# kmaninis/OSVOS-PyTorch

Measured on NVIDIA H100. Metric: frames/sec at 480x854 fwd-only, batch 1 per GPU (OSVOS.forward -> 5 logit maps), higher is better.
Workload: dtype bf16x3 (split-bf16 operands, fp32 accumulate)

## Files before the change

osvos_pytorch_b200/csrc/conv_stage1_fused.cu:

```cuda
#include <stdlib.h>
#include <string.h>

#include "conv_common.cuh"

namespace osvos {

constexpr int kS1Pitch = 10;
constexpr int kS1HaloRows = kTileH + 2;
constexpr int kS1HaloPx = kS1HaloRows * kS1Pitch;
constexpr int kS1APlane = (kS1HaloPx * 128 + 1023) / 1024 * 1024;
constexpr int kS1AStage = 2 * kS1APlane;
constexpr int kS1AStages = 2;
constexpr int kS1BPlane = 64 * 128;
constexpr int kS1BStage = 2 * kS1BPlane;
constexpr int kS1BStages = 5;
constexpr int kS1W1Bytes = (64 * 27 + 64) * 4;
constexpr int kS1Builders = 96;
constexpr int kS1Smem = kS1AStages * kS1AStage + kS1BStages * kS1BStage + kS1W1Bytes + 1024 + 512;
static_assert(kS1Smem <= 227 * 1024, "stage-1 kernel exceeds the per-CTA shared memory");
static_assert(kS1Smem + 4096 < (1 << 18), "descriptor start-address field would overflow");

struct Stage1Params {
  const float* x;
  const float* w1;
  const float* b1;
};

__global__ void __launch_bounds__(kConvThreads, 1)
conv_stage1_fused_kernel(const __grid_constant__ CUtensorMap map_w_hi, const __grid_constant__ CUtensorMap map_w_lo,
                         const Stage1Params s1, const ConvParams p) {
  extern __shared__ uint8_t smem_raw[];
  uint8_t* smem = reinterpret_cast<uint8_t*>((reinterpret_cast<uintptr_t>(smem_raw) + 1023) & ~uintptr_t(1023));
  uint8_t* smem_a = smem;
  uint8_t* smem_b = smem_a + kS1AStages * kS1AStage;
  float* w1s = reinterpret_cast<float*>(smem_b + kS1BStages * kS1BStage);
  uint64_t* bars = reinterpret_cast<uint64_t*>(reinterpret_cast<uint8_t*>(w1s) + kS1W1Bytes);
  uint64_t* a_full = bars;
  uint64_t* a_empty = bars + 2;
  uint64_t* b_full = bars + 4;
  uint64_t* b_empty = bars + 4 + kS1BStages;

  const int warp = threadIdx.x >> 5;
  const int lane = threadIdx.x & 31;

  if (threadIdx.x == 0) {
    tma_prefetch_desc(&map_w_hi);
    tma_prefetch_desc(&map_w_lo);
    for (int i = 0; i < 2; ++i) {
      mbar_init(&a_full[i], kS1Builders);
      mbar_init(&a_empty[i], 2);
    }
    for (int i = 0; i < kS1BStages; ++i) {
      mbar_init(&b_full[i], 1);
      mbar_init(&b_empty[i], 2);
    }
    fence_barrier_init();
  }
  pdl_wait();
  pdl_launch_dependents();
  for (int i = threadIdx.x; i < 64 * 27 + 64; i += kConvThreads)
    w1s[i] = i < 64 * 27 ? __ldg(s1.w1 + i) : (s1.b1 ? __ldg(s1.b1 + i - 64 * 27) : 0.f);
  __syncthreads();

  if (warp == 0) {
    if (elect_one()) {
      int b_stage = 0;
      uint32_t b_phase = 0;
      for (int tile = blockIdx.x; tile < p.total_tiles; tile += gridDim.x) {
#pragma unroll
        for (int tap = 0; tap < 9; ++tap) {
          mbar_wait(&b_empty[b_stage], b_phase ^ 1);
          uint8_t* st = smem_b + b_stage * kS1BStage;
          mbar_arrive_expect_tx(&b_full[b_stage], kS1BStage);
          tma_load_3d(&map_w_hi, &b_full[b_stage], st, 0, 0, tap);
          tma_load_3d(&map_w_lo, &b_full[b_stage], st + kS1BPlane, 0, 0, tap);
          if (++b_stage == kS1BStages) {
            b_stage = 0;
            b_phase ^= 1;
          }
        }
      }
    }
    __syncwarp();
  } else if (warp < 4) {
    const int t = threadIdx.x - 32;
    const size_t plane_sz = static_cast<size_t>(p.h) * p.w;
    int a_stage = 0;
    uint32_t a_phase = 0;
    for (int tile = blockIdx.x; tile < p.total_tiles; tile += gridDim.x) {
      int nb, tx, ty, img;
      decode_tile(p, tile, nb, tx, ty, img);
      mbar_wait(&a_empty[a_stage], a_phase ^ 1);
      uint8_t* st = smem_a + a_stage * kS1AStage;
      for (int pix = t; pix < kS1HaloPx; pix += kS1Builders) {
        const int hy = pix / kS1Pitch, hx = pix - hy * kS1Pitch;
        const int y = ty * kTileH - 1 + hy, xx = tx * kTileW - 1 + hx;
        const bool inside = y >= 0 && y < p.h && xx >= 0 && xx < p.w;
        float v[27];
#pragma unroll
        for (int ci = 0; ci < 3; ++ci) {
          const float* pl = s1.x + (static_cast<size_t>(img) * 3 + ci) * plane_sz;
#pragma unroll
          for (int r = 0; r < 3; ++r) {
            const int iy = y + r - 1;
#pragma unroll
            for (int s = 0; s < 3; ++s) {
              const int ix = xx + s - 1;
              v[ci * 9 + r * 3 + s] =
                  (inside && iy >= 0 && iy < p.h && ix >= 0 && ix < p.w) ? __ldg(pl + static_cast<size_t>(iy) * p.w + ix) : 0.f;
            }
          }
        }
#pragma unroll 1
        for (int chunk = 0; chunk < 8; ++chunk) {
          float f[8];
#pragma unroll
          for (int e = 0; e < 8; ++e) {
            const int co = chunk * 8 + e;
            float acc = w1s[64 * 27 + co];
#pragma unroll
            for (int k = 0; k < 27; ++k) acc = fmaf(w1s[co * 27 + k], v[k], acc);
            f[e] = inside ? fmaxf(acc, 0.f) : 0.f;
          }
          uint32_t hi[4], lo[4];
#pragma unroll
          for (int e = 0; e < 4; ++e) split_pack2(f[2 * e], f[2 * e + 1], hi[e], lo[e]);
          const uint32_t off = sw128_offset(pix, chunk);
          *reinterpret_cast<uint4*>(st + off) = make_uint4(hi[0], hi[1], hi[2], hi[3]);
          *reinterpret_cast<uint4*>(st + kS1APlane + off) = make_uint4(lo[0], lo[1], lo[2], lo[3]);
        }
      }
      fence_proxy_async_smem();
      mbar_arrive(&a_full[a_stage]);
      if (++a_stage == kS1AStages) {
        a_stage = 0;
        a_phase ^= 1;
      }
    }
  } else {
    const int wg = (warp - 4) >> 2, wl = warp & 3;
    const bool leader = (threadIdx.x & 127) == 0;
    constexpr uint64_t kDescA = desc_template(16, kS1Pitch * 128, kDescSW128);
    constexpr uint64_t kDescB = desc_template(16, 1024, kDescSW128);
    const uint32_t smem_a_u32 = smem_u32(smem_a) + wg * 8 * kS1Pitch * 128, smem_b_u32 = smem_u32(smem_b);
    float acc[64];
    int a_stage = 0, b_stage = 0;
    uint32_t a_phase = 0, b_phase = 0;
    StageRelease pending;
    for (int tile = blockIdx.x; tile < p.total_tiles; tile += gridDim.x) {
#pragma unroll
      for (int i = 0; i < 64; ++i) acc[i] = 0.f;
      mbar_wait(&a_full[a_stage], a_phase);
      const uint64_t da0 = kDescA | static_cast<uint64_t>((smem_a_u32 + a_stage * kS1AStage) >> 4);
#pragma unroll
      for (int tap = 0; tap < 9; ++tap) {
        const uint32_t tap_off = static_cast<uint32_t>(((tap / 3) * kS1Pitch + (tap % 3)) * (128 >> 4));
        mbar_wait(&b_full[b_stage], b_phase);
        const uint64_t db_hi = kDescB | static_cast<uint64_t>((smem_b_u32 + b_stage * kS1BStage) >> 4);
        const uint64_t da_hi = da0 + tap_off;
        const uint64_t da_lo = da_hi + (kS1APlane >> 4);
        wgmma_fence();
#pragma unroll
        for (int k = 0; k < kBlockK / 16; ++k) {
          wgmma_bf16<128>(acc, da_hi + 2 * k, db_hi + 2 * k, 1);
          wgmma_bf16<64>(acc, da_lo + 2 * k, db_hi + 2 * k, 1);
        }
        wgmma_commit();
        wgmma_wait<1>();
        pending.release(leader);
        pending.bar_b = &b_empty[b_stage];
        if (tap == 8) pending.bar_a = &a_empty[a_stage];
        if (++b_stage == kS1BStages) {
          b_stage = 0;
          b_phase ^= 1;
        }
      }
      if (++a_stage == kS1AStages) {
        a_stage = 0;
        a_phase ^= 1;
      }
      wgmma_wait<0>();
      wgmma_fence_operands(acc);
      pending.release(leader);
      conv_epilogue<64, true, true>(p, acc, tile, wg, wl, lane);
    }
  }
}

}

using namespace osvos;

extern "C" int osvos_stage1_fused(const osvos_stage1_args* a, osvos_stream_t stream_) {
  OSVOS_CHECK_ARG(a != nullptr && a->x != nullptr && a->w1 != nullptr && a->w2_packed != nullptr);
  OSVOS_CHECK_ARG(a->n > 0 && a->h > 0 && a->w > 0 && a->h <= 65535 && a->n <= 65535);
  OSVOS_CHECK_ARG((a->y_hi != nullptr && a->y_lo != nullptr) || (a->pool_hi != nullptr && a->pool_lo != nullptr));
  OSVOS_CHECK_ARG((a->y_hi == nullptr) == (a->y_lo == nullptr) && (a->pool_hi == nullptr) == (a->pool_lo == nullptr));
  {
    const uintptr_t any = reinterpret_cast<uintptr_t>(a->y_hi) | reinterpret_cast<uintptr_t>(a->y_lo) |
                          reinterpret_cast<uintptr_t>(a->pool_hi) | reinterpret_cast<uintptr_t>(a->pool_lo);
    OSVOS_CHECK_ARG((any & 3) == 0);
    OSVOS_CHECK_ARG(((reinterpret_cast<uintptr_t>(a->b1) | reinterpret_cast<uintptr_t>(a->b2) |
                      reinterpret_cast<uintptr_t>(a->w2_packed)) & 15) == 0);
  }
  cudaStream_t stream = static_cast<cudaStream_t>(stream_);
  osvos_conv3x3_args c;
  memset(&c, 0, sizeof(c));
  c.w_packed = a->w2_packed;
  c.bias = a->b2;
  c.y_hi = a->y_hi;
  c.y_lo = a->y_lo;
  c.pool_hi = a->pool_hi;
  c.pool_lo = a->pool_lo;
  c.n = a->n, c.h = a->h, c.w = a->w, c.cin = 64, c.cout = 64;
  c.flags = OSVOS_FLAG_RELU;
  ConvParams p;
  fill_conv_params(p, &c, 64);
  CUtensorMap mw_hi, mw_lo;
  int rc = encode_weight_maps(&mw_hi, &mw_lo, &c, 64);
  if (rc) return rc;
  Stage1Params s1;
  s1.x = a->x;
  s1.w1 = a->w1;
  s1.b1 = a->b1;
  const int sms = device_sm_count();
  const int grid = p.total_tiles < sms ? p.total_tiles : sms;
  auto kern = conv_stage1_fused_kernel;
  static uint64_t attr_done = 0;
  OSVOS_CHECK_CUDA(ensure_dynamic_smem(kern, kS1Smem, &attr_done));
  OSVOS_CHECK_CUDA(launch_pdl(kern, dim3(grid), dim3(kConvThreads), kS1Smem, stream, mw_hi, mw_lo, s1, p));
  return OSVOS_OK;
}
```

Before: 656.0.

## Compute conv1_1 on tensor cores inside consumer warpgroups with ping-pong tiles

Replaces the scalar-FMA builder warps that computed the 3-channel first convolution with a register-sourced wgmma (split bf16x3) inside each consumer warpgroup. The two consumer warpgroups now alternate whole tiles, ping-pong style, and are sequenced through named barriers. Producer warps give up registers via setmaxnreg, and the B pipeline grows to 7 stages. The aim is to remove the CUDA-core FMA bottleneck of building the halo activations, at the cost of more complex synchronisation and ablation flags in the hot path.

```diff
diff --git a/osvos_pytorch_b200/csrc/conv_stage1_fused.cu b/osvos_pytorch_b200/csrc/conv_stage1_fused.cu
--- a/osvos_pytorch_b200/csrc/conv_stage1_fused.cu
+++ b/osvos_pytorch_b200/csrc/conv_stage1_fused.cu
@@ -8,17 +8,19 @@
 constexpr int kS1Pitch = 10;
 constexpr int kS1HaloRows = kTileH + 2;
 constexpr int kS1HaloPx = kS1HaloRows * kS1Pitch;
+constexpr int kS1Blocks = (kS1HaloPx + 63) / 64;
 constexpr int kS1APlane = (kS1HaloPx * 128 + 1023) / 1024 * 1024;
 constexpr int kS1AStage = 2 * kS1APlane;
 constexpr int kS1AStages = 2;
 constexpr int kS1BPlane = 64 * 128;
 constexpr int kS1BStage = 2 * kS1BPlane;
-constexpr int kS1BStages = 5;
-constexpr int kS1W1Bytes = (64 * 27 + 64) * 4;
-constexpr int kS1Builders = 96;
+constexpr int kS1BStages = 7;
+constexpr int kS1W1Bytes = 2 * 64 * 128;
 constexpr int kS1Smem = kS1AStages * kS1AStage + kS1BStages * kS1BStage + kS1W1Bytes + 1024 + 512;
 static_assert(kS1Smem <= 227 * 1024, "stage-1 kernel exceeds the per-CTA shared memory");
 static_assert(kS1Smem + 4096 < (1 << 18), "descriptor start-address field would overflow");
+static_assert(kS1AStage % 1024 == 0 && kS1BStage % 1024 == 0 && kS1W1Bytes % 1024 == 0,
+              "operands keep 1024-byte alignment");
 
 struct Stage1Params {
   const float* x;
@@ -26,19 +28,37 @@
   const float* b1;
 };
 
+__device__ __forceinline__ void wgmma_bf16_rs64(float* d, const uint32_t (&a)[4], uint64_t desc_b, uint32_t scale_d) {
+  asm volatile(
+      "{\n.reg .pred p;\nsetp.ne.b32 p, %37, 0;\n"
+      "wgmma.mma_async.sync.aligned.m64n64k16.f32.bf16.bf16 {%0, %1, %2, %3, %4, %5, %6, %7, %8, %9, %10, %11, %12, %13, "
+      "%14, %15, %16, %17, %18, %19, %20, %21, %22, %23, %24, %25, %26, %27, %28, %29, %30, %31}, {%32, %33, %34, %35}, "
+      "%36, p, 1, 1, 0;\n}\n"
+      : "+f"(d[0]), "+f"(d[1]), "+f"(d[2]), "+f"(d[3]), "+f"(d[4]), "+f"(d[5]), "+f"(d[6]), "+f"(d[7]), "+f"(d[8]),
+        "+f"(d[9]), "+f"(d[10]), "+f"(d[11]), "+f"(d[12]), "+f"(d[13]), "+f"(d[14]), "+f"(d[15]), "+f"(d[16]),
+        "+f"(d[17]), "+f"(d[18]), "+f"(d[19]), "+f"(d[20]), "+f"(d[21]), "+f"(d[22]), "+f"(d[23]), "+f"(d[24]),
+        "+f"(d[25]), "+f"(d[26]), "+f"(d[27]), "+f"(d[28]), "+f"(d[29]), "+f"(d[30]), "+f"(d[31])
+      : "r"(a[0]), "r"(a[1]), "r"(a[2]), "r"(a[3]), "l"(desc_b), "r"(scale_d)
+      : "memory");
+}
+
+__device__ __forceinline__ void pin_regs(uint32_t (&r)[4]) {
+#pragma unroll
+  for (int i = 0; i < 4; ++i) asm volatile("" : "+r"(r[i])::"memory");
+}
+
 __global__ void __launch_bounds__(kConvThreads, 1)
 conv_stage1_fused_kernel(const __grid_constant__ CUtensorMap map_w_hi, const __grid_constant__ CUtensorMap map_w_lo,
                          const Stage1Params s1, const ConvParams p) {
+  constexpr int SB = kS1BStages;
   extern __shared__ uint8_t smem_raw[];
   uint8_t* smem = reinterpret_cast<uint8_t*>((reinterpret_cast<uintptr_t>(smem_raw) + 1023) & ~uintptr_t(1023));
   uint8_t* smem_a = smem;
   uint8_t* smem_b = smem_a + kS1AStages * kS1AStage;
-  float* w1s = reinterpret_cast<float*>(smem_b + kS1BStages * kS1BStage);
-  uint64_t* bars = reinterpret_cast<uint64_t*>(reinterpret_cast<uint8_t*>(w1s) + kS1W1Bytes);
-  uint64_t* a_full = bars;
-  uint64_t* a_empty = bars + 2;
-  uint64_t* b_full = bars + 4;
-  uint64_t* b_empty = bars + 4 + kS1BStages;
+  uint8_t* smem_w1 = smem_b + SB * kS1BStage;
+  uint64_t* bars = reinterpret_cast<uint64_t*>(smem_w1 + kS1W1Bytes);
+  uint64_t* b_full = bars;
+  uint64_t* b_empty = bars + SB;
 
   const int warp = threadIdx.x >> 5;
   const int lane = threadIdx.x & 31;
@@ -46,35 +66,54 @@
   if (threadIdx.x == 0) {
     tma_prefetch_desc(&map_w_hi);
     tma_prefetch_desc(&map_w_lo);
-    for (int i = 0; i < 2; ++i) {
-      mbar_init(&a_full[i], kS1Builders);
-      mbar_init(&a_empty[i], 2);
-    }
-    for (int i = 0; i < kS1BStages; ++i) {
+    for (int i = 0; i < SB; ++i) {
       mbar_init(&b_full[i], 1);
-      mbar_init(&b_empty[i], 2);
+      mbar_init(&b_empty[i], 1);
     }
     fence_barrier_init();
   }
   pdl_wait();
   pdl_launch_dependents();
-  for (int i = threadIdx.x; i < 64 * 27 + 64; i += kConvThreads)
-    w1s[i] = i < 64 * 27 ? __ldg(s1.w1 + i) : (s1.b1 ? __ldg(s1.b1 + i - 64 * 27) : 0.f);
+  for (int i = threadIdx.x; i < 64 * 4; i += kConvThreads) {
+    const int co = i >> 2, chunk = i & 3;
+    uint32_t hi[4], lo[4];
+#pragma unroll
+    for (int t = 0; t < 4; ++t) {
+      const int k0 = chunk * 8 + 2 * t;
+      const float v0 = k0 < 27 ? s1.w1[co * 27 + k0] : 0.f;
+      const float v1 = k0 + 1 < 27 ? s1.w1[co * 27 + k0 + 1] : 0.f;
+      __nv_bfloat16 h0, l0, h1, l1;
+      split_bf16(v0, h0, l0);
+      split_bf16(v1, h1, l1);
+      hi[t] = pack_bf16x2(h0, h1);
+      lo[t] = pack_bf16x2(l0, l1);
+    }
+    *reinterpret_cast<uint4*>(smem_w1 + sw128_offset(co, chunk)) = make_uint4(hi[0], hi[1], hi[2], hi[3]);
+    *reinterpret_cast<uint4*>(smem_w1 + 64 * 128 + sw128_offset(co, chunk)) = make_uint4(lo[0], lo[1], lo[2], lo[3]);
+  }
+  fence_proxy_async_smem();
   __syncthreads();
 
-  if (warp == 0) {
+  if (warp < 4) {
+    setmaxnreg_dec<40>();
+    if (warp != 0) return;
     if (elect_one()) {
+      const bool skip_b = (p.ablate & 1) != 0;
       int b_stage = 0;
       uint32_t b_phase = 0;
       for (int tile = blockIdx.x; tile < p.total_tiles; tile += gridDim.x) {
 #pragma unroll
         for (int tap = 0; tap < 9; ++tap) {
           mbar_wait(&b_empty[b_stage], b_phase ^ 1);
-          uint8_t* st = smem_b + b_stage * kS1BStage;
-          mbar_arrive_expect_tx(&b_full[b_stage], kS1BStage);
-          tma_load_3d(&map_w_hi, &b_full[b_stage], st, 0, 0, tap);
-          tma_load_3d(&map_w_lo, &b_full[b_stage], st + kS1BPlane, 0, 0, tap);
-          if (++b_stage == kS1BStages) {
+          if (skip_b) {
+            mbar_arrive(&b_full[b_stage]);
+          } else {
+            uint8_t* st = smem_b + b_stage * kS1BStage;
+            mbar_arrive_expect_tx(&b_full[b_stage], kS1BStage);
+            tma_load_3d(&map_w_hi, &b_full[b_stage], st, 0, 0, tap);
+            tma_load_3d(&map_w_lo, &b_full[b_stage], st + kS1BPlane, 0, 0, tap);
+          }
+          if (++b_stage == SB) {
             b_stage = 0;
             b_phase ^= 1;
           }
@@ -82,108 +121,166 @@
       }
     }
     __syncwarp();
-  } else if (warp < 4) {
-    const int t = threadIdx.x - 32;
-    const size_t plane_sz = static_cast<size_t>(p.h) * p.w;
-    int a_stage = 0;
-    uint32_t a_phase = 0;
-    for (int tile = blockIdx.x; tile < p.total_tiles; tile += gridDim.x) {
+    return;
+  }
+  setmaxnreg_inc<232>();
+  const int wg = (warp - 4) >> 2, wl = warp & 3;
+  const int t = threadIdx.x & 127;
+  const bool leader = t == 0;
+  const int build_bar = 3 + wg;
+  const bool skip_build = (p.ablate & 2) != 0, skip_mma = (p.ablate & 4) != 0;
+  uint8_t* stage = smem_a + wg * kS1AStage;
+  const uint32_t stage_u32 = smem_u32(stage);
+  const uint64_t dw1_hi = make_smem_desc(smem_w1, 16, 1024, kDescSW128), dw1_lo = dw1_hi + ((64 * 128) >> 4);
+  constexpr uint64_t kDescA = desc_template(16, kS1Pitch * 128, kDescSW128);
+  constexpr uint64_t kDescB = desc_template(16, 1024, kDescSW128);
+  constexpr uint32_t kLoPlaneA = kS1APlane >> 4;
+  constexpr uint32_t kHalfA = (8 * kS1Pitch * 128) >> 4;
+  const uint64_t da0 = kDescA | static_cast<uint64_t>(stage_u32 >> 4);
+  const uint32_t smem_b_u32 = smem_u32(smem_b);
+  const size_t plane_sz = static_cast<size_t>(p.h) * p.w;
+  const int q = lane & 3;
+
+  float acc[2][64];
+  StageRelease pending;
+  for (int k = wg;; k += 2) {
+    const int tile = static_cast<int>(blockIdx.x) + k * static_cast<int>(gridDim.x);
+    if (tile >= p.total_tiles) break;
+    const bool has_next = tile + static_cast<int>(gridDim.x) < p.total_tiles;
+    const int b_seq = 9 * k;
+    int b_stage = b_seq % SB;
+    uint32_t b_phase = (b_seq / SB) & 1;
+
+    if (!skip_build) {
       int nb, tx, ty, img;
       decode_tile(p, tile, nb, tx, ty, img);
-      mbar_wait(&a_empty[a_stage], a_phase ^ 1);
-      uint8_t* st = smem_a + a_stage * kS1AStage;
-      for (int pix = t; pix < kS1HaloPx; pix += kS1Builders) {
-        const int hy = pix / kS1Pitch, hx = pix - hy * kS1Pitch;
-        const int y = ty * kTileH - 1 + hy, xx = tx * kTileW - 1 + hx;
-        const bool inside = y >= 0 && y < p.h && xx >= 0 && xx < p.w;
-        float v[27];
-#pragma unroll
-        for (int ci = 0; ci < 3; ++ci) {
-          const float* pl = s1.x + (static_cast<size_t>(img) * 3 + ci) * plane_sz;
-#pragma unroll
-          for (int r = 0; r < 3; ++r) {
-            const int iy = y + r - 1;
-#pragma unroll
-            for (int s = 0; s < 3; ++s) {
-              const int ix = xx + s - 1;
-              v[ci * 9 + r * 3 + s] =
-                  (inside && iy >= 0 && iy < p.h && ix >= 0 && ix < p.w) ? __ldg(pl + static_cast<size_t>(iy) * p.w + ix) : 0.f;
-            }
-          }
-        }
+      const int py = ty * kTileH - 1, px = tx * kTileW - 1;
+      const float* img_x = s1.x + static_cast<size_t>(img) * 3 * plane_sz;
+      float v[2][8];
+      auto load_block = [&](int blk) {
+#pragma unroll
+        for (int rr = 0; rr < 2; ++rr) {
+          const int pix = 64 * blk + 16 * wl + (lane >> 2) + 8 * rr;
+          const int hy = pix / kS1Pitch, hx = pix - hy * kS1Pitch;
+          const int y = py + hy, x = px + hx;
+          const bool live = pix < kS1HaloPx && y >= 0 && y < p.h && x >= 0 && x < p.w;
+#pragma unroll
+          for (int i = 0; i < 8; ++i) {
+            const int kk = 16 * (i >> 2) + 8 * ((i >> 1) & 1) + 2 * q + (i & 1);
+            const int ci = kk / 9, rs = kk - 9 * ci, r = rs / 3, sx = rs - 3 * r;
+            const int iy = y + r - 1, ix = x + sx - 1;
+            v[rr][i] = (kk < 27 && live && iy >= 0 && iy < p.h && ix >= 0 && ix < p.w)
+                           ? __ldg(img_x + ci * plane_sz + static_cast<size_t>(iy) * p.w + ix)
+                           : 0.f;
+          }
+        }
+      };
+      load_block(0);
 #pragma unroll 1
-        for (int chunk = 0; chunk < 8; ++chunk) {
-          float f[8];
-#pragma unroll
-          for (int e = 0; e < 8; ++e) {
-            const int co = chunk * 8 + e;
-            float acc = w1s[64 * 27 + co];
-#pragma unroll
-            for (int k = 0; k < 27; ++k) acc = fmaf(w1s[co * 27 + k], v[k], acc);
-            f[e] = inside ? fmaxf(acc, 0.f) : 0.f;
-          }
-          uint32_t hi[4], lo[4];
-#pragma unroll
-          for (int e = 0; e < 4; ++e) split_pack2(f[2 * e], f[2 * e + 1], hi[e], lo[e]);
-          const uint32_t off = sw128_offset(pix, chunk);
-          *reinterpret_cast<uint4*>(st + off) = make_uint4(hi[0], hi[1], hi[2], hi[3]);
-          *reinterpret_cast<uint4*>(st + kS1APlane + off) = make_uint4(lo[0], lo[1], lo[2], lo[3]);
+      for (int blk = 0; blk < kS1Blocks; ++blk) {
+        uint32_t a_hi[2][4], a_lo[2][4];
+#pragma unroll
+        for (int ks = 0; ks < 2; ++ks)
+#pragma unroll
+          for (int f = 0; f < 4; ++f) {
+            const int rr = f & 1, h = f >> 1;
+            __nv_bfloat16 h0, l0, h1, l1;
+            split_bf16(v[rr][4 * ks + 2 * h], h0, l0);
+            split_bf16(v[rr][4 * ks + 2 * h + 1], h1, l1);
+            a_hi[ks][f] = pack_bf16x2(h0, h1);
+            a_lo[ks][f] = pack_bf16x2(l0, l1);
+          }
+#pragma unroll
+        for (int ks = 0; ks < 2; ++ks) {
+          pin_regs(a_hi[ks]);
+          pin_regs(a_lo[ks]);
+        }
+        float a1[32];
+#pragma unroll
+        for (int i = 0; i < 32; ++i) a1[i] = 0.f;
+        wgmma_fence_operands(a1);
+        wgmma_fence();
+        if (!skip_mma) {
+#pragma unroll
+          for (int ks = 0; ks < 2; ++ks) {
+            wgmma_bf16_rs64(a1, a_lo[ks], dw1_hi + 2 * ks, ks > 0 ? 1 : 0);
+            wgmma_bf16_rs64(a1, a_hi[ks], dw1_lo + 2 * ks, 1);
+            wgmma_bf16_rs64(a1, a_hi[ks], dw1_hi + 2 * ks, 1);
+          }
+        }
+        wgmma_commit();
+        if (blk + 1 < kS1Blocks) load_block(blk + 1);
+        wgmma_wait<0>();
+        wgmma_fence_operands(a1);
+#pragma unroll
+        for (int hrow = 0; hrow < 2; ++hrow) {
+          const int pix = 64 * blk + 16 * wl + (lane >> 2) + 8 * hrow;
+          if (pix >= kS1HaloPx) continue;
+          const int hy = pix / kS1Pitch, hx = pix - hy * kS1Pitch;
+          const int y = py + hy, x = px + hx;
+          const bool inside = y >= 0 && y < p.h && x >= 0 && x < p.w;
+#pragma unroll
+          for (int j = 0; j < 8; ++j) {
+            const float2 b = s1.b1 ? __ldg(reinterpret_cast<const float2*>(s1.b1 + 8 * j + 2 * (lane & 3)))
+                                   : make_float2(0.f, 0.f);
+            float f0 = b.x, f1 = b.y;
+            f0 += a1[4 * j + 2 * hrow];
+            f1 += a1[4 * j + 2 * hrow + 1];
+            f0 = fmaxf(f0, 0.f);
+            f1 = fmaxf(f1, 0.f);
+            uint32_t hi, lo;
+            split_pack2(f0, f1, hi, lo);
+            if (!inside) hi = lo = 0u;
+            const uint32_t off = sw128_offset(pix, j) + 4 * (lane & 3);
+            st_shared_u32(stage_u32 + off, hi);
+            st_shared_u32(stage_u32 + kS1APlane + off, lo);
+          }
         }
       }
       fence_proxy_async_smem();
-      mbar_arrive(&a_full[a_stage]);
-      if (++a_stage == kS1AStages) {
-        a_stage = 0;
-        a_phase ^= 1;
+      named_bar_sync(build_bar, 128);
+    }
+
+    if (k > 0) named_bar_sync(1 + wg, 256);
+#pragma unroll
+    for (int h = 0; h < 2; ++h)
+#pragma unroll
+      for (int i = 0; i < 64; ++i) acc[h][i] = 0.f;
+#pragma unroll
+    for (int h = 0; h < 2; ++h) wgmma_fence_operands(acc[h]);
+#pragma unroll
+    for (int tap = 0; tap < 9; ++tap) {
+      const uint32_t tap_off = static_cast<uint32_t>(((tap / 3) * kS1Pitch + (tap % 3)) * (128 >> 4));
+      mbar_wait(&b_full[b_stage], b_phase);
+      if (tap == 8 && has_next) named_bar_arrive(1 + (wg ^ 1), 256);
+      const uint64_t db_hi = kDescB | static_cast<uint64_t>((smem_b_u32 + b_stage * kS1BStage) >> 4);
+      wgmma_fence();
+#pragma unroll
+      for (int h = 0; h < 2; ++h) {
+        const uint64_t da_hi = da0 + h * kHalfA + tap_off;
+        const uint64_t da_lo = da_hi + kLoPlaneA;
+        if (skip_mma) continue;
+#pragma unroll
+        for (int ks = 0; ks < kBlockK / 16; ++ks) {
+          wgmma_bf16<128>(acc[h], da_hi + 2 * ks, db_hi + 2 * ks, 1);
+          wgmma_bf16<64>(acc[h], da_lo + 2 * ks, db_hi + 2 * ks, 1);
+        }
       }
-    }
-  } else {
-    const int wg = (warp - 4) >> 2, wl = warp & 3;
-    const bool leader = (threadIdx.x & 127) == 0;
-    constexpr uint64_t kDescA = desc_template(16, kS1Pitch * 128, kDescSW128);
-    constexpr uint64_t kDescB = desc_template(16, 1024, kDescSW128);
-    const uint32_t smem_a_u32 = smem_u32(smem_a) + wg * 8 * kS1Pitch * 128, smem_b_u32 = smem_u32(smem_b);
-    float acc[64];
-    int a_stage = 0, b_stage = 0;
-    uint32_t a_phase = 0, b_phase = 0;
-    StageRelease pending;
-    for (int tile = blockIdx.x; tile < p.total_tiles; tile += gridDim.x) {
-#pragma unroll
-      for (int i = 0; i < 64; ++i) acc[i] = 0.f;
-      mbar_wait(&a_full[a_stage], a_phase);
-      const uint64_t da0 = kDescA | static_cast<uint64_t>((smem_a_u32 + a_stage * kS1AStage) >> 4);
-#pragma unroll
-      for (int tap = 0; tap < 9; ++tap) {
-        const uint32_t tap_off = static_cast<uint32_t>(((tap / 3) * kS1Pitch + (tap % 3)) * (128 >> 4));
-        mbar_wait(&b_full[b_stage], b_phase);
-        const uint64_t db_hi = kDescB | static_cast<uint64_t>((smem_b_u32 + b_stage * kS1BStage) >> 4);
-        const uint64_t da_hi = da0 + tap_off;
-        const uint64_t da_lo = da_hi + (kS1APlane >> 4);
-        wgmma_fence();
-#pragma unroll
-        for (int k = 0; k < kBlockK / 16; ++k) {
-          wgmma_bf16<128>(acc, da_hi + 2 * k, db_hi + 2 * k, 1);
-          wgmma_bf16<64>(acc, da_lo + 2 * k, db_hi + 2 * k, 1);
-        }
-        wgmma_commit();
-        wgmma_wait<1>();
-        pending.release(leader);
-        pending.bar_b = &b_empty[b_stage];
-        if (tap == 8) pending.bar_a = &a_empty[a_stage];
-        if (++b_stage == kS1BStages) {
-          b_stage = 0;
-          b_phase ^= 1;
-        }
+      wgmma_commit();
+      wgmma_wait<1>();
+      pending.release(leader);
+      pending.bar_b = &b_empty[b_stage];
+      if (++b_stage == SB) {
+        b_stage = 0;
+        b_phase ^= 1;
       }
-      if (++a_stage == kS1AStages) {
-        a_stage = 0;
-        a_phase ^= 1;
-      }
-      wgmma_wait<0>();
-      wgmma_fence_operands(acc);
-      pending.release(leader);
-      conv_epilogue<64, true, true>(p, acc, tile, wg, wl, lane);
-    }
+    }
+    wgmma_wait<0>();
+#pragma unroll
+    for (int h = 0; h < 2; ++h) wgmma_fence_operands(acc[h]);
+    pending.release(leader);
+#pragma unroll
+    for (int h = 0; h < 2; ++h) conv_epilogue<64, true, true>(p, acc[h], tile, h, wl, lane);
   }
 }
 
```

Measured after the change: 652.7 (median of 6 runs). About the same (-0.5%).
